# blackpigg/MCMTT_OPTICALFLOW

Hardware: AMD Instinct MI355X
Metric: Tracker2D frames/sec (all cameras) + achieved HBM GB/s fraction, 1/2/4/8 GPU (higher is better)
Workload: dtype u8+f32

## Files before the change

include/psn_lk.h:

```cpp
#ifndef PSN_LK_H
#define PSN_LK_H

#include <stddef.h>
#include <stdint.h>

#ifdef __cplusplus
extern "C" {
#endif

#define PSN_LK_ABI_VERSION 5

#define PSN_LK_OK 0
#define PSN_LK_ERR_ARG (-1)
#define PSN_LK_ERR_WINSIZE (-2)
#define PSN_LK_ERR_HIP (-3)
#define PSN_LK_ERR_NOMEM (-4)
#define PSN_LK_ERR_SLOT (-5)
#define PSN_LK_ERR_LEVEL_CAP (-6)
#define PSN_LK_ERR_COMM (-7)
#define PSN_LK_ERR_UNSUPPORTED (-8)

#define PSN_LK_USE_INITIAL_FLOW 4
#define PSN_LK_GET_MIN_EIGENVALS 8
#define PSN_LK_ACCUM_SCALAR 0x100
// ... 54 lines not shown
int psn_lk_track(psn_lk_ctx *ctx, const psn_lk_query *q, int nq, const float *prev_xy, float *next_xy,
                 uint8_t *status, float *err);
int psn_lk_track_device(psn_lk_ctx *ctx, const psn_lk_query *q, int nq, const float *d_prev_xy,
                        float *d_next_xy, uint8_t *d_status, float *d_err);

int psn_lk_track_device_counted(psn_lk_ctx *ctx, const psn_lk_query *q, int nq, const int *d_counts,
                                const float *d_prev_xy, float *d_next_xy, uint8_t *d_status, float *d_err);
int psn_lk_track_device_counted_strided(psn_lk_ctx *ctx, const psn_lk_query *q, int nq, const int *d_counts,
                                        int count_stride, const float *d_prev_xy, float *d_next_xy, uint8_t *d_status,
                                        float *d_err);

int psn_calc_optical_flow_pyr_lk(psn_lk_ctx *ctx, const uint8_t *prev_img, const uint8_t *next_img,
                                 int stride, const float *prev_pts, float *next_pts, uint8_t *status,
                                 float *err, int npts, const psn_lk_params *params);

int psn_lk_read_level(psn_lk_ctx *ctx, int slot, int level, uint8_t *host, int stride);
int psn_lk_level_size(psn_lk_ctx *ctx, int level, int *w, int *h);

int psn_lk_enable_timing(psn_lk_ctx *ctx, int capacity, int every);
int psn_lk_timing_stats(psn_lk_ctx *ctx, int *n_push, double *push_ms, int *n_track, double *track_ms);
int psn_lk_timing_launches(psn_lk_ctx *ctx, int cap, double *ms, int *tag, int *n);

#define PSN_LK_VARIANT_THREADS 1
#define PSN_LK_VARIANT_GENERIC 2
#define PSN_LK_VARIANT_ONEWAVE 3
#define PSN_LK_VARIANT_BOX 4
#define PSN_LK_VARIANT_TILED_LDS 5
#define PSN_LK_VARIANT_FUSED_HELPERS 6
#define PSN_LK_VARIANT_LARGE 7
#define PSN_LK_VARIANT_LG_LDS 8
#define PSN_LK_VARIANT_LG_JR 9
#define PSN_LK_VARIANT_ST_OVL 10
#define PSN_LK_VARIANT_POISON_LDS 11
int psn_lk_debug_set_variant(psn_lk_ctx *ctx, int key, int value);

int psn_lk_debug_count_samples(psn_lk_ctx *ctx, int on);
int psn_lk_debug_read_samples(psn_lk_ctx *ctx, unsigned long long *out);

int psn_lk_debug_set_stamps(psn_lk_ctx *ctx, void *d_stamps);

typedef struct psn_gridfast_params {
    int threshold;
    int nonmax;
    int max_total;
    int grid_rows;
    int grid_cols;
    int cap;
} psn_gridfast_params;
void psn_gridfast_default_params(psn_gridfast_params *p);
int psn_gridfast_detect(psn_lk_ctx *ctx, int slot, const int *rois, int nroi, const psn_gridfast_params *p,
                        uint32_t seed, float *out_xy, int *out_count, int *out_total);
int psn_gridfast_detect_device(psn_lk_ctx *ctx, int slot, const int *rois, int nroi, const psn_gridfast_params *p,
                               uint32_t seed, float *d_out_xy, int *d_out_count, int *d_out_total);
int psn_gridfast_detect_device_sets(psn_lk_ctx *ctx, int nset, const int *slots, const int *nrois, const int *rois,
                                    const psn_gridfast_params *p, uint32_t seed, float *d_out_xy, int *d_out_count,
                                    int *d_out_total);

#define PSN_RGBHIST_BINS 16
typedef struct psn_rgbhist_rect {
    const uint8_t *frame;
    int stride;
    int x, y, w, h;
} psn_rgbhist_rect;
int psn_rgbhist_device(const psn_rgbhist_rect *d_rects, int nrect, uint32_t *d_counts, void *hip_stream);
int psn_lk_box_histograms(psn_lk_ctx *ctx, int nset, const int *slots, const int *nrects, const int *rects,
                          uint32_t *counts);
// ... 19 lines not shown
```

mcmtt_opticalflow_amd/_lib.py:

```python
from __future__ import annotations

import ctypes
import os
import re

_HERE = os.path.dirname(os.path.abspath(__file__))
LIB_PATH = os.path.join(_HERE, "lib", "libpsn_lk.so")
STAMPS_LIB_PATH = os.path.join(_HERE, "lib", "libpsn_lk_stamps.so")
HEADER_PATH = os.path.join(os.path.dirname(_HERE), "include", "psn_lk.h")
HEADER_PATHS = [HEADER_PATH] + [os.path.join(os.path.dirname(_HERE), "include", h)
                                for h in ("psn_sgsmooth.h", "psn_t2d_device.h", "psn_jpeg.h")]

PSN_LK_OK = 0
ERRORS = {
    -1: "PSN_LK_ERR_ARG",
    -2: "PSN_LK_ERR_WINSIZE",
    -3: "PSN_LK_ERR_HIP",
    -4: "PSN_LK_ERR_NOMEM",
    -5: "PSN_LK_ERR_SLOT",
    -6: "PSN_LK_ERR_LEVEL_CAP",
    -7: "PSN_LK_ERR_COMM",
    -8: "PSN_LK_ERR_UNSUPPORTED",
}
USE_INITIAL_FLOW = 4
GET_MIN_EIGENVALS = 8
ACCUM_SCALAR = 0x100
OVERLAP_OFF, OVERLAP_STREAM, OVERLAP_FUSED = 0, 1, 2
TERM_COUNT = 1
TERM_EPS = 2
MAX_WIN_WIDTH = 6400
COMM_UNIQUE_ID_BYTES = 128
VARIANTS = {"threads": 1, "generic": 2, "onewave": 3, "box": 4, "tiled_lds": 5, "fused_helpers": 6,
            "large": 7, "lg_lds": 8, "lg_jr": 9, "st_ovl": 10, "poison_lds": 11}


class PsnLkError(RuntimeError):
    def __init__(self, code: int, msg: str = ""):
        self.code = code
        super().__init__(f"{ERRORS.get(code, code)}: {msg}")


class LkParams(ctypes.Structure):
    _fields_ = [
        ("win_w", ctypes.c_int),
        ("win_h", ctypes.c_int),
        ("max_level", ctypes.c_int),
        ("term_type", ctypes.c_int),
        ("max_count", ctypes.c_int),
        ("epsilon", ctypes.c_double),
        ("flags", ctypes.c_int),
        ("min_eig_threshold", ctypes.c_double),
    ]


class LkQuery(ctypes.Structure):
    _fields_ = [
        ("prev_slot", ctypes.c_int),
        ("next_slot", ctypes.c_int),
        ("first_pt", ctypes.c_int),
        ("num_pts", ctypes.c_int),
        ("params", LkParams),
    ]


class GridFastParams(ctypes.Structure):
    _fields_ = [
# ... 164 lines not shown
```

mcmtt_opticalflow_amd/csrc/psn_lk_abi.cpp:

```cpp
#include <hip/hip_runtime.h>
#include <hsa/hsa.h>
#include <hsa/hsa_ext_amd.h>

#include <algorithm>
#include <chrono>
#include <mutex>
#include <cstdarg>
#include <cstdio>
#include <cstdlib>
#include <cstring>
#include <new>
#include <string>
#include <vector>

#include "psn_lk.h"
#include "psn_jpeg.h"
#include "psn_gridfast.h"
#include "psn_rgbhist.h"
#include "psn_lk_kernels.h"

using psn::LevelDev;

struct psn_lk_ctx {
    int device = 0;
// ... 33 lines not shown
    struct ColorSrc {
        const uint8_t *p = nullptr;
        int stride = 0, channels = 0;
        bool shared = false;
        unsigned gen = 0;
    };
    std::vector<ColorSrc> color_src;
    unsigned src_gen = 0;
    hipStream_t hist_stream = nullptr;
    hipEvent_t hist_ev = nullptr;
    psn_rgbhist_rect *h_hist_rects = nullptr;
    psn_rgbhist_rect *d_hist_rects = nullptr;
    uint32_t *h_hist_counts = nullptr;
    uint32_t *d_hist_counts = nullptr;
    size_t hist_cap = 0;
    psn_jpeg_ctx *jpeg = nullptr;
    uint8_t *d_pyr = nullptr;
    LevelDev *d_slots = nullptr;
    std::vector<LevelDev> h_slots;
    std::vector<char> filled;
    uint8_t *d_src = nullptr;
    size_t d_src_cap = 0;
    float *d_prev = nullptr, *d_next = nullptr, *d_err = nullptr;
    uint8_t *d_status = nullptr;
    size_t d_pts_cap = 0;
    int force_threads = 0;
    bool force_generic = false;
    bool onewave = true;
#ifndef PSN_ST_OVL_DEFAULT
#define PSN_ST_OVL_DEFAULT 1
#endif
    bool st_ovl = PSN_ST_OVL_DEFAULT != 0;
    bool poison_lds = false;
    bool box = true;
    int tiled_lds = 76 * 1024;
    int num_cus = 256;
    bool force_large = false;
    int lg_lds = 24 * 1024;
    bool lg_jr = true;
    struct LgWs {
        hipStream_t s = nullptr;
        void *p = nullptr;
        size_t bytes = 0;
        hipEvent_t done = nullptr;
    };
    std::vector<LgWs> lg_ws;
    std::vector<void *> lg_retired;
    unsigned long long *d_stamps = nullptr;
    unsigned long long *d_samples = nullptr;
    bool count_samples = false;
    uint32_t *d_gf_kp = nullptr;
    int *d_gf_cnt = nullptr;
    size_t gf_kp_cap = 0, gf_cnt_cap = 0;
    float *d_gf_xy = nullptr;
    int *d_gf_oc = nullptr, *d_gf_ot = nullptr;
    size_t gf_out_cap = 0;
    int gf_nroi_cap = 0;
    int tcap = 0;
    std::vector<hipEvent_t> ev_push, ev_track;
    std::vector<int> track_tag;
    long n_push = 0, n_track = 0;
    long calls_push = 0, calls_track = 0;
    int every = 1;
    std::string err;
};

// ... 870 lines not shown
        bool builds = false;
        if (c->pend && fused_slot < 0 && !d_counts) {
            int tx, ty, plds;
            psn::pyramid_grid(c->pend_args, tx, ty, plds);
            a.pyr = c->pend_args;
            a.pyr_ntiles = tx * ty;
            a.pyr_tiles_x = tx;
            a.pyr_ctr = c->d_ctr;
            const int helpers = std::min(c->fused_helpers, a.pyr_ntiles);
            a.lk_wgs = wgs;
            a.total_wgs = wgs + helpers;
            wgs += helpers;
            lds = std::max(lds, psn::kStScratchBytes + plds);
            c->pend = false;
            fused_slot = c->pend_slot;
            builds = true;
        }
        a.poison_lds = c->poison_lds ? lds : 0;
        HIPCHK(c, psn::launch_lk_st(a, wgs, nt, ept, ow_e, occ, lds, c->stream));
        return builds ? mark_fused_build(c, fused_slot) : PSN_LK_OK;
    }
    if (cls == kClsBx) {
        const int upt = key / 10;
        const bool notail = key % 10 != 0;
        int lds_bx = 0;
        for (int i = 0; i < a.nq; i++) {
            psn::LkQueryDev &d = a.q[i];
            d.bx_hw = 1;
            while (d.bx_hw < 8 && psn::BxLayout(d.win_w, d.win_h, upt, d.bx_hw + 1).total <= psn::bx_lds_target(upt, notail))
                d.bx_hw++;
            lds_bx = std::max(lds_bx, psn::BxLayout(d.win_w, d.win_h, upt, d.bx_hw).total);
        }
        a.poison_lds = c->poison_lds ? lds_bx : 0;
        HIPCHK(c, psn::launch_lk_bx(a, wgs, upt, notail, lds_bx, c->stream));
        return PSN_LK_OK;
    }
    if (cls == kClsTiled) {
        int threads = maxpx <= 1024 ? 64 : maxpx <= 4096 ? 128 : 256;
        if (forced == 64 || forced == 128 || forced == 256) threads = forced;
        lds = 0;
        for (int i = 0; i < a.nq; i++) lds = std::max(lds, psn::lk_lds_bytes(a.q[i].win_w, a.q[i].win_h, a.q[i].tile_rows));
        HIPCHK(c, psn::launch_lk(a, wgs, threads, lds, c->stream));
        return PSN_LK_OK;
    }
    long long slot = 0;
    lds = 0;
    for (int i = 0; i < a.nq; i++) {
        slot = std::max(slot, psn::lg_slot_int2(a.q[i].win_w, a.q[i].win_h));
        lds = std::max(lds, psn::lg_lds_bytes(a.q[i].win_w, a.q[i].win_h, a.q[i].tile_rows, a.q[i].lg_jr != 0, key));
    }
    const size_t slot_bytes = (size_t)slot * 8;
    const long long fit = std::max<long long>((long long)(kLgWsBudget / slot_bytes), 1);
    const int grid = (int)std::min<long long>(wgs, fit);
    void *ws = nullptr;
    int rc = ensure_lg_ws(c, slot_bytes * grid, &ws);
    if (rc) return rc;
    a.lg_ws = (int2 *)ws;
    a.lg_slot = slot;
    a.lk_wgs = wgs;
    a.total_wgs = wgs;
    a.poison_lds = c->poison_lds ? lds : 0;
    HIPCHK(c, psn::launch_lk_lg(a, grid, lds, key, c->stream));
    for (auto &e : c->lg_ws)
        if (e.s == c->stream) {
            if (!e.done) HIPCHK(c, hipEventCreateWithFlags(&e.done, hipEventDisableTiming));
            HIPCHK(c, hipEventRecord(e.done, c->stream));
// ... 228 lines not shown
    if (!prev_pts || !next_pts || !status) return PSN_LK_ERR_ARG;
    HIPCHK(c, hipSetDevice(c->device));
    const int sa = c->user_slots, sb = c->user_slots + 1;
    int rc = push_host_impl(c, sa, prev_img, stride, 1);
    if (rc) return rc;
    rc = push_host_impl(c, sb, next_img, stride, 1);
    if (rc) return rc;
    psn_lk_query q;
    q.prev_slot = sa;
    q.next_slot = sb;
    q.first_pt = 0;
    q.num_pts = npts;
    q.params = p;
    return track_host_impl(c, &q, 1, prev_pts, next_pts, status, err, true);
}

int psn_lk_debug_set_variant(psn_lk_ctx *c, int key, int value) {
    if (!c) return PSN_LK_ERR_ARG;
    switch (key) {
    case PSN_LK_VARIANT_THREADS:
        if (value != 0 && value != 64 && value != 128 && value != 256 && value != 512) return PSN_LK_ERR_ARG;
        c->force_threads = value;
        return PSN_LK_OK;
    case PSN_LK_VARIANT_GENERIC: c->force_generic = value != 0; return PSN_LK_OK;
    case PSN_LK_VARIANT_ONEWAVE: c->onewave = value != 0; return PSN_LK_OK;
    case PSN_LK_VARIANT_BOX: c->box = value != 0; return PSN_LK_OK;
    case PSN_LK_VARIANT_TILED_LDS: c->tiled_lds = std::max(16 * 1024, std::min(value, 160 * 1024 - 1024)); return PSN_LK_OK;
    case PSN_LK_VARIANT_FUSED_HELPERS: c->fused_helpers = std::max(0, value); return PSN_LK_OK;
    case PSN_LK_VARIANT_LARGE: c->force_large = value != 0; return PSN_LK_OK;
    case PSN_LK_VARIANT_LG_LDS: c->lg_lds = std::max(4 * 1024, std::min(value, 160 * 1024 - 1024)); return PSN_LK_OK;
    case PSN_LK_VARIANT_LG_JR: c->lg_jr = value != 0; return PSN_LK_OK;
    case PSN_LK_VARIANT_ST_OVL: c->st_ovl = value != 0; return PSN_LK_OK;
    case PSN_LK_VARIANT_POISON_LDS: c->poison_lds = value != 0; return PSN_LK_OK;
    default: return PSN_LK_ERR_ARG;
    }
}

int psn_lk_debug_count_samples(psn_lk_ctx *c, int on) {
    if (!c) return PSN_LK_ERR_ARG;
    HIPCHK(c, hipSetDevice(c->device));
    if (on) {
        if (!c->d_samples) HIPCHK(c, hipMalloc(&c->d_samples, sizeof(unsigned long long)));
        HIPCHK(c, hipDeviceSynchronize());
        HIPCHK(c, hipMemset(c->d_samples, 0, sizeof(unsigned long long)));
    }
    c->count_samples = on != 0;
    return PSN_LK_OK;
}

int psn_lk_debug_read_samples(psn_lk_ctx *c, unsigned long long *out) {
    if (!c || !out) return PSN_LK_ERR_ARG;
    *out = 0;
    if (!c->d_samples) return PSN_LK_OK;
    HIPCHK(c, hipSetDevice(c->device));
    HIPCHK(c, hipDeviceSynchronize());
    HIPCHK(c, hipMemcpy(out, c->d_samples, sizeof(unsigned long long), hipMemcpyDeviceToHost));
    return PSN_LK_OK;
}

int psn_lk_debug_set_stamps(psn_lk_ctx *c, void *d_stamps) {
    if (!c) return PSN_LK_ERR_ARG;
#ifdef PSN_LK_STAMPS
    c->d_stamps = (unsigned long long *)d_stamps;
    return PSN_LK_OK;
#else
    (void)d_stamps;
// ... 273 lines not shown
```

mcmtt_opticalflow_amd/csrc/psn_lk_kernels.h:

```cpp
#pragma once

#include <hip/hip_runtime.h>
#include <stdint.h>

#include "psn_lk.h"

namespace psn {

constexpr int kMaxLevels = PSN_LK_MAX_LEVELS;
constexpr int kMaxQueries = 32;
constexpr int kJMargin = 3;
constexpr int kPyrMaxTop = 5;

struct LevelDev {
    uint8_t *p;
    int w, h, pitch;
    int pad_;
};

struct PyrBuildArgs {
    const uint8_t *src;
    int src_stride;
    int channels;
    int nlevels;
// ... 26 lines not shown
    int sub_pts, sub_pstride;
};
__device__ __forceinline__ int lk_query_point(const LkQueryDev &Q, const int *counts, int count_stride, int g) {
    int loc = g - Q.wg_begin;
    if (Q.sub_pts > 0) {
        const int sub = loc / Q.sub_pts;
        loc -= sub * Q.sub_pts;
        if (counts && loc >= counts[Q.qidx + sub * count_stride]) return -1;
        return Q.pt_begin + sub * Q.sub_pstride + loc;
    }
    if (counts && loc >= counts[Q.qidx]) return -1;
    return Q.pt_begin + loc;
}
__host__ __device__ inline unsigned div_magic(int d) { return d > 0 ? ((1u << 22) + (unsigned)d - 1u) / (unsigned)d : 0u; }

struct RingGeo {
    uint8_t *base;
    long long slot_bytes;
    long long off[kMaxLevels];
    int w[kMaxLevels], h[kMaxLevels], pitch[kMaxLevels];
};

struct LkLaunchArgs {
    const LevelDev *slots;
    RingGeo ring;
    const float *prev;
    float *next;
    uint8_t *status;
    float *err;
    unsigned long long *stamps;
    unsigned long long *samples;
    int nq;
    int poison_lds;
    const int *counts;
    int count_stride;
    LkQueryDev q[kMaxQueries];
    int pyr_ntiles, pyr_tiles_x;
    int total_wgs, lk_wgs;
    unsigned *pyr_ctr;
    PyrBuildArgs pyr;
    int2 *lg_ws;
    long long lg_slot;
};

__host__ __device__ constexpr int align16(int x) { return (x + 15) & ~15; }
__host__ __device__ inline int lk_jreg_w(int w) { return w + 1 + 2 * kJMargin; }
__host__ __device__ inline int lk_jreg_h(int h) { return h + 1 + 2 * kJMargin; }
__host__ __device__ inline int lk_off_dw(int w, int h) { return align16(2 * w * h); }
__host__ __device__ inline int lk_off_jr(int w, int h) { return lk_off_dw(w, h) + align16(4 * w * h); }
__host__ __device__ inline int lk_off_red(int w, int h) { return lk_off_jr(w, h) + align16(lk_jreg_w(w) * lk_jreg_h(h)); }
constexpr int kRedBytes = 256;
__host__ __device__ inline int lk_off_tile(int w, int h) { return lk_off_red(w, h) + kRedBytes; }
__host__ __device__ inline int lk_tile_pimg_bytes(int w, int tr) { return align16((tr + 3) * (w + 3)); }
__host__ __device__ inline int lk_tile_dg_bytes(int w, int tr) { return align16(4 * (tr + 1) * (w + 1)); }
__host__ __device__ inline int lk_tile_prod_bytes(int w, int tr) { return 12 * (tr * w + 20); }
__host__ __device__ inline int lk_lds_bytes(int w, int h, int tr) {
    return lk_off_tile(w, h) + lk_tile_pimg_bytes(w, tr) + lk_tile_dg_bytes(w, tr) + lk_tile_prod_bytes(w, tr);
}

__host__ __device__ inline int round16i(int x) { return (x + 15) & ~15; }
__host__ __device__ inline int lk_st_planeA(int w, int h, bool sse) {
    const int n = sse ? w / 4 : 0;
    return 4 * round16i(h * n) + round16i(h * (w - 4 * n) + 1);
}
__host__ __device__ inline int lk_st_planeB(int w, int h, bool sse) {
    const int n = sse ? w / 8 : 0;
// ... 56 lines not shown
            iw = dg + nlev * dg_stride;
            r = iw + nlev * iw_stride;
            ra = r;
            int rb = rb_a;
            if (rb < pb) rb = pb;
            if (rb < eb) rb = eb;
            total = r + rb;
        }
    }
};
constexpr int kBxNT = 256;
constexpr int kBxMaxUPT = 16;
constexpr int kBxRecInts = 8 * 15 + 4;
constexpr int kBxXInts = 2 * 4 * kBxRecInts;
constexpr int kBxScrBytes = (kBxXInts + 32) * 4 + 64;
constexpr int kBxMaxLds = 64 * 1024;
constexpr int kBxMaxLds2 = 80 * 1024;
constexpr int kBxLdsTarget = 53 * 1024;
__host__ __device__ constexpr int bx_occupancy(int upt, bool notail) {
    return upt <= 4 ? 4 : (upt >= 12 || (!notail && upt >= 10)) ? 2 : 3;
}
__host__ __device__ constexpr int bx_lds_target(int upt, bool notail) {
    return bx_occupancy(upt, notail) == 4 ? 40 * 1024 : bx_occupancy(upt, notail) == 3 ? kBxLdsTarget : kBxMaxLds2;
}
__host__ __device__ constexpr int bx_max_lds(int upt, bool notail) {
    return bx_occupancy(upt, notail) == 2 ? kBxMaxLds2 : kBxMaxLds;
}
__host__ __device__ inline int bx_qw(int w) { return (w + 3) >> 2; }
__host__ __device__ inline int bx_pm(int w) { return bx_qw(w) + 2; }
__host__ __device__ inline int bx_jrp(int w) { return st_jreg_w(w) + 8; }
__host__ __device__ inline int bx_round4(int x) { return (x + 3) & ~3; }
__host__ __device__ inline int bx_region(int n) { return ((n + 15) & ~15) + 4; }
__host__ __device__ inline int bx_pc(int upt) { return 128 * upt + 96; }
struct BxLayout {
    int jr, un, pb, total;
    __host__ __device__ BxLayout(int w, int h, int upt, int hw = 1) {
        jr = align16(kBxScrBytes);
        un = jr + align16(st_jreg_h(h) * bx_jrp(w));
        const int pim = align16((h + 3) * 4 * bx_pm(w));
        const int planes = 24 * bx_pc(upt) * hw;
        pb = pim > planes ? pim : planes;
        total = un + pb + 1024;
    }
};
inline int bx_err_rows(int w, int h, int pb) {
    for (int t = h; t >= 1; t--)
        if (4 * bx_round4(t * w) <= pb) return t;
    return 1;
}

constexpr int kLgNT = 256;
constexpr int kLgTQs[2] = {192, 128};
constexpr int kLgTQNoJr = 128;
constexpr int kLgTQE = 128;
__host__ __device__ constexpr int lg_sreg(int tq) { return ((tq + 15) & ~15) + 4; }
__host__ __device__ constexpr int lg_plane(int tq) { return 4 * lg_sreg(tq) + ((4 * tq + 15) & ~15) + 4; }
__host__ __device__ constexpr int lg_scr_bytes() { return align16((kBxXInts + 32) * 4); }
__host__ __device__ constexpr int lg_tiles_a_bytes(int tq) { return 2 * 3 * lg_plane(tq) * 4 + 1024; }
__host__ __device__ constexpr int lg_tiles_b_bytes(int tq) { return 2 * 2 * lg_plane(tq) * 4 + 1024; }
__host__ __device__ inline int lg_band_bytes(int w, int tr) { return align16((tr + 3) * 4 * bx_pm(w)); }
__host__ __device__ inline int lg_jr_bytes(int w, int h) { return align16(st_jreg_h(h) * bx_jrp(w)); }
#ifndef PSN_LG_XB
#define PSN_LG_XB 0
#endif
constexpr int kXbRecBytes = 10 * 256 * 8;
#ifndef PSN_LG_POOL_KB
// ... 68 lines not shown
```

mcmtt_opticalflow_amd/csrc/psn_lk_kernels.hip:

```cpp
#include <float.h>
#include <limits.h>

#include <type_traits>

#include "psn_gridfast.h"
#include "psn_lk_kernels.h"
#include "psn_lk_device.h"
#include "psn_lk_bx.h"

namespace psn {


#define LK_STAMP(slot) PSN_STAMP(A.stamps, threadIdx.x == 0, (size_t)blockIdx.x * 64 + (slot))
#define LK_COUNT(slot, v) PSN_STAMP_VAL(A.stamps, threadIdx.x == 0, (size_t)blockIdx.x * 64 + (slot), v)




__device__ __forceinline__ uint8_t load_src(const PyrBuildArgs &a, int y, int x) {
    const uint8_t *row = a.src + (size_t)y * a.src_stride;
    if (a.channels == 1) return row[x];
    const uint8_t *p = row + 3 * x;
    return (uint8_t)((p[0] * 1868 + p[1] * 9617 + p[2] * 4899 + (1 << 13)) >> 14);
}
// ... 1671 lines not shown
        A.status[pi] = (uint8_t)status;
        if (A.err) A.err[pi] = errv;
    }
    if (A.pyr_ntiles > 0) pyr_tail<NT>(A, smem);
}

template <int UPT, bool NOTAIL>
__global__ __launch_bounds__(kBxNT, bx_occupancy(UPT, NOTAIL)) void lk_kernel_bx(LkLaunchArgs A) {
    extern __shared__ __attribute__((aligned(16))) uint8_t smem[];
    static_assert(UPT % 2 == 0, "units are processed in pairs");
    constexpr int NT = kBxNT;
    const int tid = threadIdx.x, lane = tid & 63;
    if (A.poison_lds) lds_poison<NT>(smem, A.poison_lds);
    const int g = xcd_remap((int)blockIdx.x, (int)gridDim.x);
    int qi = 0;
    while (qi + 1 < A.nq && g >= A.q[qi + 1].wg_begin) qi++;
    const LkQueryDev &Q = A.q[qi];
    const int pi = lk_query_point(Q, A.counts, A.count_stride, g);
    if (pi < 0) return;
    const int w = Q.win_w, h = Q.win_h;
    const int maxL = Q.max_level, flags = Q.flags;
    const bool sse = (flags & PSN_LK_ACCUM_SCALAR) == 0;
    const int QW = bx_qw(w), U = h * QW;
    const int nqB = sse ? (w / 8) * 2 : 0, n8 = 4 * nqB, tB = w - n8;
    const int nqA = sse ? w / 4 : 0, nA4 = 4 * nqA, tA = w - nA4;
    const int PM = bx_pm(w), JRW = st_jreg_w(w), JRH = st_jreg_h(h), JRP = bx_jrp(w), JRP4 = JRP >> 2;
    const BxLayout lay(w, h, UPT);
    int *X = (int *)smem;
    float *RS = (float *)(X + kBxXInts);
    int *EP = (int *)(RS + 16);
    volatile int *FLG = (volatile int *)(RS + 24);
    if (threadIdx.x < 7) FLG[threadIdx.x] = threadIdx.x < 6 ? -1 : 0;
    int fb_epoch = 0;
    uint8_t *JR = smem + lay.jr;
    const uint32_t *JR32 = (const uint32_t *)JR;
    uint8_t *UN = smem + lay.un;
    const uint32_t *P32 = (const uint32_t *)UN;
    float *PL = (float *)UN;

    const int u0 = tid * UPT;
    const int y0 = u0 / QW, q0 = u0 - y0 * QW;
    unsigned UB[UPT / 2];
    unsigned sseB = 0;
    {
        int y = y0, q = q0;
#pragma unroll
        for (int k = 0; k < UPT; k++) {
            const unsigned o = u0 + k < U ? (unsigned)(y * JRP + 4 * q) : 0u;
            if (k & 1)
                UB[k >> 1] |= o << 16;
            else
                UB[k >> 1] = o;
            sseB |= (unsigned)(q < nqB) << k;
            if (++q == QW) {
                q = 0;
                y++;
            }
        }
    }

    const float hwx = __fmul_rn((float)(w - 1), 0.5f), hwy = __fmul_rn((float)(h - 1), 0.5f);
    const float px0 = A.prev[2 * pi], py0 = A.prev[2 * pi + 1];
    float NPx = 0.f, NPy = 0.f;
    if (flags & PSN_LK_USE_INITIAL_FLOW) {
        NPx = A.next[2 * pi];
        NPy = A.next[2 * pi + 1];
    }
    int status = 1;
    float errv = 0.f;
    int par = 0;
#ifdef PSN_LK_STAMPS
    unsigned long long bx_acc[16] = {}, bx_t = 0, bx_t0 = 0, bx_r0 = 0;
    PSN_CLK_ORDERED(bx_t0);
    bx_t = bx_t0;
    asm volatile("s_memrealtime %0\n\ts_waitcnt lgkmcnt(0)" : "=s"(bx_r0) : : "memory");
#endif

    unsigned IP[UPT][2], XP[UPT][2], YP[UPT][2];
    int gmax = 0;
    unsigned nwin = 0;

    for (int level = maxL; level >= 0; level--) {
        const LevelDev I = ring_level_u(A.ring, Q.prev_slot, level);
        const LevelDev J = ring_level_u(A.ring, Q.next_slot, level);
        const int cols = I.w, rows = I.h;
        const float scale = ldexpf(1.f, -level);
        float px = __fmul_rn(px0, scale), py = __fmul_rn(py0, scale);
        float nx, ny;
        if (level == maxL) {
            if (flags & PSN_LK_USE_INITIAL_FLOW) {
                nx = __fmul_rn(NPx, scale);
                ny = __fmul_rn(NPy, scale);
            } else {
                nx = px;
                ny = py;
            }
        } else {
            nx = __fmul_rn(NPx, 2.f);
            ny = __fmul_rn(NPy, 2.f);
        }
        NPx = nx;
        NPy = ny;
        px = __fsub_rn(px, hwx);
        py = __fsub_rn(py, hwy);
        const int ipx = cv_floor(px), ipy = cv_floor(py);
        if (win_outside(ipx, ipy, w, h, cols, rows)) {
            if (level == 0) {
                status = 0;
                errv = 0.f;
            }
            continue;
        }
        int iw00, iw01, iw10, iw11;
        bilin_weights(__fsub_rn(px, (float)ipx), __fsub_rn(py, (float)ipy), iw00, iw01, iw10, iw11);
        nx = __fsub_rn(nx, hwx);
        ny = __fsub_rn(ny, hwy);
        int jr_x0 = (cv_floor(nx) - kStJMargin) & ~3, jr_y0 = cv_floor(ny) - kStJMargin;

        __syncthreads();
        dma_patch<NT>(UN, I, ipy - 1, ipx - 1, w + 3, h + 3, PM, Q.dv_bxpm);
        dma_wait();
        dma_patch<NT>(JR, J, jr_y0, jr_x0, JRW, JRH, JRP4, Q.dv_bxjr);
        barrier_inflight();
        PSN_PH_MARK(bx_acc, bx_t, 0);
        bx_prio_lo();

        float sA[3];
        nwin++;
        {
            const int sh = (ipx - 1) & 3;
            int T11[5] = {0, 0, 0, 0, 0}, T22[5] = {0, 0, 0, 0, 0}, T12[5] = {0, 0, 0, 0, 0};
            int M12[5] = {0, 0, 0, 0, 0}, m12[5] = {0, 0, 0, 0, 0};
            int gmx = 0, gmn = 0;
            const bool interior = ipx >= 0 && ipy >= 0 && ipx + 4 * QW + 2 <= cols && ipy + h + 1 <= rows;
            const int c256 = 1 << 8, c8192 = 1 << 13;
            auto apass = [&](auto inner) {
            constexpr bool IN = decltype(inner)::value;
            int y = y0, q = q0;
            asm volatile("" : "+v"(y), "+v"(q));
#pragma unroll
            for (int k = 0; k < UPT; k++) {
                const bool uv = u0 + k < U;
                const int yy = uv ? y : 0, qq = uv ? q : 0;
                bx_unit<IN, NOTAIL>(P32, PM, sh, yy, qq, uv, w, ipx, ipy, cols, rows, iw00, iw01, iw10, iw11, c256,
                                    c8192, IP[k], XP[k], YP[k], gmx, gmn);
                asm volatile("" : "+v"(IP[k][0]), "+v"(IP[k][1]), "+v"(XP[k][0]), "+v"(XP[k][1]), "+v"(YP[k][0]),
                             "+v"(YP[k][1]), "+v"(gmx), "+v"(gmn));
                if (++q == QW) {
                    q = 0;
                    y++;
                }
                __builtin_amdgcn_sched_barrier(0);
            }
            };
            if (interior)
                apass(std::true_type());
            else
                apass(std::false_type());
            gmax = max(gmx, -gmn);
            int q = q0;
// ... 39 lines not shown
                            T22[4] = mad16p<1, 1>(yt[u][hh], yt[u][hh], mad16p<0, 0>(yt[u][hh], yt[u][hh], T22[4]));
                            const int ta = mad16p<0, 0>(xt[u][hh], yt[u][hh], T12[4]);
                            const int tb = mad16p<1, 1>(xt[u][hh], yt[u][hh], ta);
                            run2(T12[4], M12[4], m12[4], ta, tb);
                        }
                }
                asm volatile("" : "+v"(T11[0]), "+v"(T11[1]), "+v"(T11[2]), "+v"(T11[3]), "+v"(T11[4]), "+v"(T22[0]),
                             "+v"(T22[1]), "+v"(T22[2]), "+v"(T22[3]), "+v"(T22[4]));
                asm volatile("" : "+v"(T12[0]), "+v"(T12[1]), "+v"(T12[2]), "+v"(T12[3]), "+v"(T12[4]), "+v"(M12[0]),
                             "+v"(M12[1]), "+v"(M12[2]), "+v"(M12[3]), "+v"(M12[4]));
                asm volatile("" : "+v"(m12[0]), "+v"(m12[1]), "+v"(m12[2]), "+v"(m12[3]), "+v"(m12[4]));
            }
            int T[15], M[15], m[15];
#pragma unroll
            for (int c = 0; c < 5; c++) {
                T[c] = T11[c], M[c] = T11[c], m[c] = 0;
                T[5 + c] = T12[c], M[5 + c] = M12[c], m[5 + c] = m12[c];
                T[10 + c] = T22[c], M[10 + c] = T22[c], m[10 + c] = 0;
            }
            PSN_PH_MARK(bx_acc, bx_t, 1);
            bx_prio_hi();
            int *rec = X + par * 4 * kBxRecInts;
            par ^= 1;
            bx_publish<15>(T, rec, NOTAIL || tA == 0);
            dma_wait();
            __syncthreads();
            bx_check<15>(T, M, m, false, rec, NOTAIL || tA == 0);
            __syncthreads();
            int tot, h0, base0;
            const bool exact = bx_eval<15>(rec, tot, h0, base0);
            if (exact) {
#pragma unroll
                for (int s = 0; s < 3; s++) sA[s] = combine_a5([&](int i) { return rl_f(tot, i); }, s, sse);
            } else {
                int ftid = (int)threadIdx.x;
                asm volatile("" : "+v"(ftid));
                const int HW = Q.bx_hw, PCA = 3 * bx_pc(UPT) * HW;
                const bool chl = ftid < 15;
                const int cl = chl ? ftid : 0, cs = cl / 5, cc = cl - 5 * cs;
                float acc = (float)base0;
                const int g_last = (U - 1) / (32 * UPT);
                auto geoA = [&](int g, int &sa, int &ta, int &nsse, int &ntail) {
                    const int ua = 32 * UPT * g, ub = min(ua + 32 * UPT * HW, U);
                    sa = (ua / QW) * nqA + min(ua % QW, nqA);
                    ta = (ua / QW) * tA + min(max(4 * (ua % QW) - nA4, 0), tA);
                    nsse = (ub / QW) * nqA + min(ub % QW, nqA) - sa;
                    ntail = (ub / QW) * tA + min(max(4 * (ub % QW) - nA4, 0), tA) - ta;
                };
                auto unitA = [&](int yk, int qk, bool uv, unsigned x0, unsigned x1, unsigned y0_, unsigned y1_, float *buf,
                                 int S, int P, int sa, int ta) {
                    if (!uv) return;
                    unsigned xp[2] = {x0, x1}, yp[2] = {y0_, y1_};
                    asm volatile("" : "+v"(xp[0]), "+v"(xp[1]), "+v"(yp[0]), "+v"(yp[1]));
                    const bool su = NOTAIL || qk < nqA;
                    const int base = su ? yk * nqA + qk - sa : 4 * S + yk * tA + 4 * qk - nA4 - ta;
#pragma unroll
                    for (int i = 0; i < 4; i++) {
                        const int gx = (i & 1) ? hi16(xp[i >> 1]) : lo16(xp[i >> 1]);
                        const int gy = (i & 1) ? hi16(yp[i >> 1]) : lo16(yp[i >> 1]);
                        const bool on = 4 * qk + i < w;
                        float *d1 = on ? buf + (su ? i * S + base : base + i) : PL + 2 * PCA;
                        const int pp = on ? P : 1;
                        d1[0] = (float)__mul24(gx, gx);
                        d1[pp] = (float)__mul24(gx, gy);
                        d1[2 * pp] = (float)__mul24(gy, gy);
                    }
// ... 108 lines not shown
                    for (int i = len; i < ((len + 15) & ~15); i++) rg[i] = 0.f;
                };
                writeA(h0, PL);
                padA(h0, PL);
                __syncthreads();
                for (int g = h0, t = 0; g <= g_last; g += HW, t ^= 1) {
                    float *cur = PL + t * PCA, *nxt = PL + (t ^ 1) * PCA;
                    if (g + HW <= g_last) writeA(g + HW, nxt);
                    if ((ftid >> 6) == 0) {
                        int sa, ta, nsse, ntail;
                        geoA(g, sa, ta, nsse, ntail);
                        const int S = bx_region(nsse), P = 4 * S + bx_region(ntail);
                        const int len = chl ? (cc < 4 ? nsse : ntail) : 0;
                        const int nbmax = NOTAIL ? (nsse + 15) >> 4 : __builtin_amdgcn_readlane(wave_max_scan((len + 15) >> 4), 63);
                        if (chl && (!NOTAIL || cc < 4)) acc = chain_sum_pl<NOTAIL>(cur + cs * P + cc * S, len, nbmax, acc);
                        if (g + HW <= g_last) padA(g + HW, nxt);
                    }
                    __syncthreads();
                }
                if (ftid < 64) {
#pragma unroll
                    for (int s = 0; s < 3; s++) {
                        const float t = combine_a5([&](int i) { return readlane_f(acc, i); }, s, sse);
                        if (ftid == 0) RS[s] = t;
                    }
                }
                __syncthreads();
                sA[0] = RS[0];
                sA[1] = RS[1];
                sA[2] = RS[2];
            }
            PSN_PH_MARK(bx_acc, bx_t, 2);
        }
        const LkSolve S = lk_solve(sA[0], sA[1], sA[2], w * h, Q.min_eig);
        if (flags & PSN_LK_GET_MIN_EIGENVALS) errv = S.minEig;
        if (!S.ok) {
            if (level == 0) status = 0;
            continue;
        }

        float pdx = 0.f, pdy = 0.f;
        for (int j = 0; j < Q.max_count; j++) {
            const int inx = cv_floor(nx), iny = cv_floor(ny);
            if (win_outside(inx, iny, w, h, cols, rows)) {
                if (level == 0) status = 0;
                break;
            }
            int w00, w01, w10, w11;
            bilin_weights(__fsub_rn(nx, (float)inx), __fsub_rn(ny, (float)iny), w00, w01, w10, w11);
            if (!(jr_covers(inx, iny, w, h, jr_x0, jr_y0, JRW, JRH))) {
                jr_x0 = (inx - kStJMargin) & ~3;
                jr_y0 = iny - kStJMargin;
                dma_patch<NT>(JR, J, jr_y0, jr_x0, JRW, JRH, JRP4, Q.dv_bxjr);
                dma_wait();
                __syncthreads();
            }
            PSN_PH_MARK(bx_acc, bx_t, 3);
            bx_prio_lo();
            PSN_PH_COUNT(bx_acc, 10);
            nwin++;
            const unsigned W0 = pack_w(w00, w01), W1 = pack_w(w10, w11);
            const int ox = inx - jr_x0, oy = iny - jr_y0, sj = ox & 3;
            const unsigned s0 = bx_sel(sj, 0), s1 = bx_sel(sj, 1), s2 = bx_sel(sj, 2), s3 = bx_sel(sj, 3);
            int T1[5] = {0, 0, 0, 0, 0}, M1[5] = {0, 0, 0, 0, 0}, m1[5] = {0, 0, 0, 0, 0};
            int T2[5] = {0, 0, 0, 0, 0}, M2[5] = {0, 0, 0, 0, 0}, m2[5] = {0, 0, 0, 0, 0};
            int dmx = 0, dmn = 0;
            const int c256 = opaque256();
            const bool dtrack = __ballot(gmax > kExact / 8160) != 0ull;
            auto bmain = [&](auto trk) {
                unsigned jo0 = (unsigned)((const uint8_t *)(JR32 + oy * JRP4 + (ox >> 2)) - smem);
                unsigned jo1 = jo0 + 4u * (unsigned)JRP4;
// ... 84 lines not shown
                    asm volatile("" : "+v"(T1[0]), "+v"(T1[1]), "+v"(T1[2]), "+v"(T1[3]), "+v"(T1[4]), "+v"(M1[0]),
                                 "+v"(M1[1]), "+v"(M1[2]), "+v"(M1[3]), "+v"(M1[4]));
                    asm volatile("" : "+v"(m1[0]), "+v"(m1[1]), "+v"(m1[2]), "+v"(m1[3]), "+v"(m1[4]), "+v"(T2[0]),
                                 "+v"(T2[1]), "+v"(T2[2]), "+v"(T2[3]), "+v"(T2[4]));
                    asm volatile("" : "+v"(M2[0]), "+v"(M2[1]), "+v"(M2[2]), "+v"(M2[3]), "+v"(M2[4]), "+v"(m2[0]),
                                 "+v"(m2[1]), "+v"(m2[2]), "+v"(m2[3]), "+v"(m2[4]), "+v"(dmx), "+v"(dmn));
                }
            };
            if (dtrack)
                bmain(std::true_type());
            else
                bmain(std::false_type());
            const int dmax = max(dmx, -dmn);
            const bool bad = (long long)dmax * gmax > (long long)kExact;
            int T[10], M[10], m[10];
#pragma unroll
            for (int c = 0; c < 5; c++) {
                T[c] = T1[c], M[c] = M1[c], m[c] = m1[c];
                T[5 + c] = T2[c], M[5 + c] = M2[c], m[5 + c] = m2[c];
            }
            PSN_PH_MARK(bx_acc, bx_t, 4);
            bx_prio_hi();
            int *rec = X + par * 4 * kBxRecInts;
            par ^= 1;
            bx_publish<10>(T, rec, NOTAIL || tB == 0);
            PSN_PH_MARK(bx_acc, bx_t, 9);
            __syncthreads();
            bx_check<10>(T, M, m, bad, rec, NOTAIL || tB == 0);
            __syncthreads();
            int tot, h0, base0;
            float b1, b2;
            const bool bex = bx_eval<10>(rec, tot, h0, base0);
            PSN_PH_MARK(bx_acc, bx_t, 5);
            if (bex) {
                combine_b10([&](int i) { return rl_f(tot, i); }, sse, b1, b2);
            } else {
                int ftid = (int)threadIdx.x;
                asm volatile("" : "+v"(ftid));
                const int HW = Q.bx_hw, PC = bx_pc(UPT) * HW;
                const bool chl = ftid < 10;
                const int cl = chl ? ftid : 0, cs = cl / 5, cc = cl - 5 * cs;
                float acc = (float)base0;
                const int g_last = (U - 1) / (32 * UPT);
                auto tile_geo = [&](int g, int &sa, int &ta, int &nsse, int &ntail) {
                    const int ua = 32 * UPT * g, ub = min(ua + 32 * UPT * HW, U);
                    sa = (ua / QW) * nqB + min(ua % QW, nqB);
                    ta = (ua / QW) * tB + min(max(4 * (ua % QW) - n8, 0), tB);
                    nsse = (ub / QW) * nqB + min(ub % QW, nqB) - sa;
                    ntail = (ub / QW) * tB + min(max(4 * (ub % QW) - n8, 0), tB) - ta;
                };
                auto tile_unit = [&](int yk, int qk, bool uv, const unsigned (&ip)[2], const unsigned (&xp)[2],
                                     const unsigned (&yp)[2], float *buf, int S, int P, int sa, int ta, int zf) {
                    if (!uv) return;
                    int d[4];
                    bx_diffs(JR32 + (oy + yk) * JRP4 + (ox >> 2) + qk, JRP4, W0, W1, s0, s1, s2, s3, ip, d, zf);
                    const bool su = NOTAIL || qk < nqB;
                    const int base = su ? yk * nqB + qk - sa : 4 * S + yk * tB + 4 * qk - n8 - ta;
#pragma unroll
                    for (int i = 0; i < 4; i++) {
                        const int gx = (i & 1) ? hi16(xp[i >> 1]) : lo16(xp[i >> 1]);
                        const int gy = (i & 1) ? hi16(yp[i >> 1]) : lo16(yp[i >> 1]);
                        const bool on = 4 * qk + i < w;
                        float *d1 = on ? buf + (su ? i * S + base : base + i) : PL + 6 * PC;
                        d1[0] = (float)__mul24(d[i], gx);
                        d1[on ? P : 1] = (float)__mul24(d[i], gy);
                    }
                };
                constexpr int K1 = UPT / 2;
                const bool split = HW == 1 && (UPT & 1) == 0;
// ... 278 lines not shown
                                if (4 * qk + i < w) PL[(yk - r0) * w + 4 * qk + i] = (float)abs(d[i]);
                        }
                        if (++qk == QW) {
                            qk = 0;
                            yk++;
                        }
                    }
                    __syncthreads();
                    if (tid == 0) acc = chain_sum(PL, tr * w, acc);
                }
                if (tid == 0) RS[8] = acc;
                __syncthreads();
                errval = RS[8];
            }
            errv = lk_err(errval, w * h);
        }
    }

#ifdef PSN_LK_STAMPS
    {
        unsigned long long t_end;
        PSN_CLK_ORDERED(t_end);
        bx_acc[15] = t_end - bx_t0;
        unsigned long long r1;
        unsigned hwid, xcc;
        asm volatile("s_memrealtime %0\n\ts_waitcnt lgkmcnt(0)" : "=s"(r1) : : "memory");
        asm volatile("s_getreg_b32 %0, hwreg(HW_REG_HW_ID)" : "=s"(hwid));
        asm volatile("s_getreg_b32 %0, hwreg(HW_REG_XCC_ID)" : "=s"(xcc));
        if (tid == 0 && A.stamps) {
            for (int i = 0; i < 16; i++) A.stamps[(size_t)g * 64 + i] = bx_acc[i];
            A.stamps[(size_t)g * 64 + 16] = bx_r0;
            A.stamps[(size_t)g * 64 + 17] = r1;
            A.stamps[(size_t)g * 64 + 18] = ((unsigned long long)xcc << 32) | hwid;
        }
    }
#endif
    if (tid == 0) {
        if (FLG[6]) {
            NPx = NPy = errv = __builtin_nanf("");
            status = 0;
        }
        A.next[2 * pi] = NPx;
        A.next[2 * pi + 1] = NPy;
        A.status[pi] = (uint8_t)status;
        if (A.err) A.err[pi] = errv;
        if (A.samples) atomicAdd(A.samples, (unsigned long long)nwin * (unsigned)(w * h));
    }
}

#define PSN_BX_KERNELS(X)                                         \
    X(4, true) X(4, false) X(8, true) X(8, false) X(10, true)     \
    X(10, false) X(12, true) X(12, false) X(16, true) X(16, false)
#define PSN_ST_KERNELS(X)                                                                 \
    X(64, 2, 0, 1) X(64, 4, 0, 1) X(128, 2, 0, 1) X(128, 4, 0, 1) X(256, 2, 0, 1)         \
    X(512, 1, 0, 1) X(512, 2, 0, 1) X(256, 2, 4, 1) X(256, 2, 7, 1) X(256, 2, 8, 1)       \
    X(256, 4, 8, 1) X(256, 2, 16, 1) X(256, 4, 16, 1) X(256, 4, 0, 1) X(256, 2, 4, 3)     \
    X(256, 2, 7, 3) X(256, 2, 8, 3)

hipError_t launch_lk_bx(const LkLaunchArgs &a, int total_wgs, int upt, bool notail, int lds_bytes, hipStream_t s) {
    if (total_wgs <= 0) return hipSuccess;
    const dim3 grid(total_wgs), block(kBxNT);
#define PSN_BX_LAUNCH(U, NOTAIL)                                                         \
    if (upt == U && notail == NOTAIL) {                                                  \
        hipLaunchKernelGGL((lk_kernel_bx<U, NOTAIL>), grid, block, lds_bytes, s, a);     \
        return hipGetLastError();                                                        \
    }
// ... 47 lines not shown
```

Baseline: 2600.

## Defer inexact A-matrix fallback and fuse it with first-iteration b-vector pass

When the fast exact path for the structure tensor (A) fails in the box LK kernel, the fallback tile reduction is now deferred and merged into the first iteration's b-vector fallback. One double-buffered LDS tile pass computes all five gradient products (gx², gxgy, gy², d·gx, d·gy) together. The goal is to avoid two separate slow tile sweeps over the window gradients on the fallback path. The change is controlled by a new default-on bx_fuse variant and a compile-time LDS-fit check. It adds code complexity, LDS usage and a different loop exit (break) when the solve fails.

After: 2612, median of 6. About the same (+0.5%).

```diff
diff --git a/include/psn_lk.h b/include/psn_lk.h
--- a/include/psn_lk.h
+++ b/include/psn_lk.h
@@ -110,6 +110,7 @@
 #define PSN_LK_VARIANT_LG_JR 9
 #define PSN_LK_VARIANT_ST_OVL 10
 #define PSN_LK_VARIANT_POISON_LDS 11
+#define PSN_LK_VARIANT_BX_FUSE 12
 int psn_lk_debug_set_variant(psn_lk_ctx *ctx, int key, int value);
 
 int psn_lk_debug_count_samples(psn_lk_ctx *ctx, int on);
diff --git a/mcmtt_opticalflow_amd/_lib.py b/mcmtt_opticalflow_amd/_lib.py
--- a/mcmtt_opticalflow_amd/_lib.py
+++ b/mcmtt_opticalflow_amd/_lib.py
@@ -31,7 +31,7 @@
 MAX_WIN_WIDTH = 6400
 COMM_UNIQUE_ID_BYTES = 128
 VARIANTS = {"threads": 1, "generic": 2, "onewave": 3, "box": 4, "tiled_lds": 5, "fused_helpers": 6,
-            "large": 7, "lg_lds": 8, "lg_jr": 9, "st_ovl": 10, "poison_lds": 11}
+            "large": 7, "lg_lds": 8, "lg_jr": 9, "st_ovl": 10, "poison_lds": 11, "bx_fuse": 12}
 
 
 class PsnLkError(RuntimeError):
diff --git a/mcmtt_opticalflow_amd/csrc/psn_lk_abi.cpp b/mcmtt_opticalflow_amd/csrc/psn_lk_abi.cpp
--- a/mcmtt_opticalflow_amd/csrc/psn_lk_abi.cpp
+++ b/mcmtt_opticalflow_amd/csrc/psn_lk_abi.cpp
@@ -89,6 +89,10 @@
 #endif
     bool st_ovl = PSN_ST_OVL_DEFAULT != 0;
     bool poison_lds = false;
+#ifndef PSN_BX_FUSE_DEFAULT
+#define PSN_BX_FUSE_DEFAULT 1
+#endif
+    bool bx_fuse = PSN_BX_FUSE_DEFAULT != 0;
     bool box = true;
     int tiled_lds = 76 * 1024;
     int num_cus = 256;
@@ -1025,6 +1029,7 @@
             lds_bx = std::max(lds_bx, psn::BxLayout(d.win_w, d.win_h, upt, d.bx_hw).total);
         }
         a.poison_lds = c->poison_lds ? lds_bx : 0;
+        a.bx_fuse = c->bx_fuse ? 1 : 0;
         HIPCHK(c, psn::launch_lk_bx(a, wgs, upt, notail, lds_bx, c->stream));
         return PSN_LK_OK;
     }
@@ -1319,6 +1324,7 @@
     case PSN_LK_VARIANT_LG_JR: c->lg_jr = value != 0; return PSN_LK_OK;
     case PSN_LK_VARIANT_ST_OVL: c->st_ovl = value != 0; return PSN_LK_OK;
     case PSN_LK_VARIANT_POISON_LDS: c->poison_lds = value != 0; return PSN_LK_OK;
+    case PSN_LK_VARIANT_BX_FUSE: c->bx_fuse = value != 0; return PSN_LK_OK;
     default: return PSN_LK_ERR_ARG;
     }
 }
diff --git a/mcmtt_opticalflow_amd/csrc/psn_lk_kernels.h b/mcmtt_opticalflow_amd/csrc/psn_lk_kernels.h
--- a/mcmtt_opticalflow_amd/csrc/psn_lk_kernels.h
+++ b/mcmtt_opticalflow_amd/csrc/psn_lk_kernels.h
@@ -82,6 +82,7 @@
     unsigned long long *samples;
     int nq;
     int poison_lds;
+    int bx_fuse;
     const int *counts;
     int count_stride;
     LkQueryDev q[kMaxQueries];
@@ -204,6 +205,11 @@
 __host__ __device__ inline int bx_round4(int x) { return (x + 3) & ~3; }
 __host__ __device__ inline int bx_region(int n) { return ((n + 15) & ~15) + 4; }
 __host__ __device__ inline int bx_pc(int upt) { return 128 * upt + 96; }
+__host__ __device__ inline int bx_fz_plane(int n) { return 4 * bx_region(n) + 4; }
+__host__ __device__ inline int bx_fz_buf(int n) { return 5 * bx_fz_plane(n); }
+__host__ __device__ constexpr bool bx_fz_build(int upt, bool notail) {
+    return notail && 48 * (128 * upt + 96) + kBxScrBytes <= bx_lds_target(upt, notail);
+}
 struct BxLayout {
     int jr, un, pb, total;
     __host__ __device__ BxLayout(int w, int h, int upt, int hw = 1) {
diff --git a/mcmtt_opticalflow_amd/csrc/psn_lk_kernels.hip b/mcmtt_opticalflow_amd/csrc/psn_lk_kernels.hip
--- a/mcmtt_opticalflow_amd/csrc/psn_lk_kernels.hip
+++ b/mcmtt_opticalflow_amd/csrc/psn_lk_kernels.hip
@@ -1727,6 +1727,11 @@
     volatile int *FLG = (volatile int *)(RS + 24);
     if (threadIdx.x < 7) FLG[threadIdx.x] = threadIdx.x < 6 ? -1 : 0;
     int fb_epoch = 0;
+    constexpr bool FZ = bx_fz_build(UPT, NOTAIL);
+    int *DA = (int *)(RS + 32);
+    auto fz_fits = [&]() {
+        return A.bx_fuse && Q.max_count > 0 && 8 * bx_fz_buf(32 * UPT) <= BxLayout(w, h, UPT, Q.bx_hw).pb;
+    };
     uint8_t *JR = smem + lay.jr;
     const uint32_t *JR32 = (const uint32_t *)JR;
     uint8_t *UN = smem + lay.un;
@@ -1765,7 +1770,7 @@
     float errv = 0.f;
     int par = 0;
 #ifdef PSN_LK_STAMPS
-    unsigned long long bx_acc[16] = {}, bx_t = 0, bx_t0 = 0, bx_r0 = 0;
+    unsigned long long bx_acc[24] = {}, bx_t = 0, bx_t0 = 0, bx_r0 = 0;
     PSN_CLK_ORDERED(bx_t0);
     bx_t = bx_t0;
     asm volatile("s_memrealtime %0\n\ts_waitcnt lgkmcnt(0)" : "=s"(bx_r0) : : "memory");
@@ -1821,6 +1826,7 @@
         bx_prio_lo();
 
         float sA[3];
+        bool defA = false;
         nwin++;
         {
             const int sh = (ipx - 1) & 3;
@@ -1926,6 +1932,11 @@
             if (exact) {
 #pragma unroll
                 for (int s = 0; s < 3; s++) sA[s] = combine_a5([&](int i) { return rl_f(tot, i); }, s, sse);
+            } else if (FZ && fz_fits() && !win_outside(cv_floor(nx), cv_floor(ny), w, h, cols, rows)) {
+                defA = true;
+                int dt = (int)threadIdx.x;
+                asm volatile("" : "+v"(dt));
+                if (dt < 16) DA[dt] = dt < 15 ? base0 : h0;
             } else {
                 int ftid = (int)threadIdx.x;
                 asm volatile("" : "+v"(ftid));
@@ -2100,11 +2111,14 @@
             }
             PSN_PH_MARK(bx_acc, bx_t, 2);
         }
-        const LkSolve S = lk_solve(sA[0], sA[1], sA[2], w * h, Q.min_eig);
-        if (flags & PSN_LK_GET_MIN_EIGENVALS) errv = S.minEig;
-        if (!S.ok) {
-            if (level == 0) status = 0;
-            continue;
+        LkSolve S = {};
+        if (!defA) {
+            S = lk_solve(sA[0], sA[1], sA[2], w * h, Q.min_eig);
+            if (flags & PSN_LK_GET_MIN_EIGENVALS) errv = S.minEig;
+            if (!S.ok) {
+                if (level == 0) status = 0;
+                continue;
+            }
         }
 
         float pdx = 0.f, pdy = 0.f;
@@ -2255,9 +2269,128 @@
             float b1, b2;
             const bool bex = bx_eval<10>(rec, tot, h0, base0);
             PSN_PH_MARK(bx_acc, bx_t, 5);
-            if (bex) {
-                combine_b10([&](int i) { return rl_f(tot, i); }, sse, b1, b2);
-            } else {
+            if (bex) combine_b10([&](int i) { return rl_f(tot, i); }, sse, b1, b2);
+            bool fzd = false;
+            if constexpr (FZ) if (defA) {
+                defA = false;
+                fzd = true;
+                int ftid = (int)threadIdx.x;
+                asm volatile("" : "+v"(ftid));
+                constexpr int K1 = UPT / 2;
+                constexpr int TU = 32 * UPT;
+                const int BUF = bx_fz_buf(TU);
+                const int t0a = DA[15], t0b = bex ? 1 << 20 : h0;
+                const int t_first = min(t0a, t0b), t_last = (U - 1) / TU;
+                const bool chl = ftid < 20;
+                const int cl = chl ? ftid : 0, cp = cl >> 2, ci = cl & 3;
+                const int bA = DA[5 * min(cp, 2) + ci];
+                const int bB = __builtin_amdgcn_ds_bpermute(4 * (5 * max(cp - 3, 0) + ci), base0);
+                const float acc0 = (float)(cp < 3 ? bA : bB);
+                const int tst = cp < 3 ? t0a : t0b;
+                float acc = acc0;
+                unsigned fo0 = (unsigned)((const uint8_t *)(JR32 + oy * JRP4 + (ox >> 2)) - smem);
+                unsigned fo1 = fo0 + 4u * (unsigned)JRP4;
+                asm volatile("" : "+s"(fo0), "+s"(fo1));
+                auto fz_write = [&](int g, float *buf, auto lowerT) {
+                    constexpr bool lower = decltype(lowerT)::value;
+                    const int zf = opaque256();
+                    const int n = min(TU, U - g * TU), S = bx_region(n), P = bx_fz_plane(n);
+                    const bool up = (ftid & 32) != 0;
+                    const int ub = lower ? (up ? (ftid ^ 32) * UPT + K1 : ftid * UPT) : (up ? ftid * UPT + K1 : (ftid ^ 32) * UPT);
+                    const int rel = ub - g * TU;
+                    const bool wb = g >= t0b;
+                    auto pick = [](unsigned a, unsigned b) {
+                        auto r = __builtin_amdgcn_permlane32_swap(a, b, false, false);
+                        return lower ? r[0] : r[1];
+                    };
+                    auto uoff = [&](int k) { return (k & 1) ? UB[k >> 1] >> 16 : UB[k >> 1] & 0xffffu; };
+#pragma unroll
+                    for (int k = 0; k < K1; k++) {
+                        const unsigned ip[2] = {pick(IP[k][0], IP[K1 + k][0]), pick(IP[k][1], IP[K1 + k][1])};
+                        unsigned xp[2] = {pick(XP[k][0], XP[K1 + k][0]), pick(XP[k][1], XP[K1 + k][1])};
+                        unsigned yp[2] = {pick(YP[k][0], YP[K1 + k][0]), pick(YP[k][1], YP[K1 + k][1])};
+                        const unsigned off = pick(uoff(k), uoff(K1 + k));
+                        if (ub + k < U) {
+                            asm volatile("" : "+v"(xp[0]), "+v"(xp[1]), "+v"(yp[0]), "+v"(yp[1]));
+                            float *d1 = buf + rel + k;
+#pragma unroll
+                            for (int i = 0; i < 4; i++) {
+                                const int gx = (i & 1) ? hi16(xp[i >> 1]) : lo16(xp[i >> 1]);
+                                const int gy = (i & 1) ? hi16(yp[i >> 1]) : lo16(yp[i >> 1]);
+                                d1[i * S] = (float)__mul24(gx, gx);
+                                d1[i * S + P] = (float)__mul24(gx, gy);
+                                d1[i * S + 2 * P] = (float)__mul24(gy, gy);
+                            }
+                            if (wb) {
+                                int d[4];
+                                bx_diffs2((const uint32_t *)(smem + fo0 + off), (const uint32_t *)(smem + fo1 + off), W0, W1,
+                                          s0, s1, s2, s3, ip, d, zf);
+#pragma unroll
+                                for (int i = 0; i < 4; i++) {
+                                    const int gx = (i & 1) ? hi16(xp[i >> 1]) : lo16(xp[i >> 1]);
+                                    const int gy = (i & 1) ? hi16(yp[i >> 1]) : lo16(yp[i >> 1]);
+                                    d1[i * S + 3 * P] = (float)__mul24(d[i], gx);
+                                    d1[i * S + 4 * P] = (float)__mul24(d[i], gy);
+                                }
+                            }
+                        }
+                    }
+                };
+                for (int g = t_first - 1, t = 1; g <= t_last; g++, t ^= 1) {
+                    float *cur = PL + t * BUF, *nxt = PL + (t ^ 1) * BUF;
+                    if (g < t_last && (ftid >> 6) == (g + 1) >> 1) {
+                        if ((g + 1) & 1)
+                            fz_write(g + 1, nxt, std::false_type());
+                        else
+                            fz_write(g + 1, nxt, std::true_type());
+                    }
+                    if (chl) {
+                        if (g >= t_first) {
+                            const int n = min(TU, U - g * TU);
+                            acc = chain_sum_pl<true>(cur + cp * bx_fz_plane(n) + ci * bx_region(n), n, (n + 15) >> 4, acc);
+                            if (g < tst) acc = acc0;
+                        }
+                        if (g < t_last) {
+                            const int n = min(TU, U - (g + 1) * TU);
+                            float *rg = nxt + cp * bx_fz_plane(n) + ci * bx_region(n);
+                            for (int i = n; i < ((n + 15) & ~15); i++) rg[i] = 0.f;
+                        }
+                    }
+                    __syncthreads();
+                }
+                PSN_PH_MARK(bx_acc, bx_t, 19);
+                PSN_PH_COUNT(bx_acc, bex ? 21 : 20);
+                if (ftid < 64) {
+                    auto ga = [&](int i) { return i % 5 == 4 ? 0.f : readlane_f(acc, 4 * (i / 5) + i % 5); };
+#pragma unroll
+                    for (int s = 0; s < 3; s++) {
+                        const float t = combine_a5(ga, s, sse);
+                        if (ftid == 0) RS[s] = t;
+                    }
+                    if (!bex) {
+                        float r1, r2;
+                        combine_b10([&](int i) { return i % 5 == 4 ? 0.f : readlane_f(acc, 12 + 4 * (i / 5) + i % 5); }, sse, r1,
+                                    r2);
+                        if (ftid == 0) {
+                            RS[4] = r1;
+                            RS[5] = r2;
+                        }
+                    }
+                }
+                __syncthreads();
+                if (!bex) {
+                    b1 = RS[4];
+                    b2 = RS[5];
+                }
+                S = lk_solve(RS[0], RS[1], RS[2], w * h, Q.min_eig);
+                if (flags & PSN_LK_GET_MIN_EIGENVALS) errv = S.minEig;
+                if (!S.ok) {
+                    if (level == 0) status = 0;
+                    nwin--;
+                    break;
+                }
+            }
+            if (!fzd && !bex) {
                 int ftid = (int)threadIdx.x;
                 asm volatile("" : "+v"(ftid));
                 const int HW = Q.bx_hw, PC = bx_pc(UPT) * HW;
@@ -2602,6 +2735,7 @@
             A.stamps[(size_t)g * 64 + 16] = bx_r0;
             A.stamps[(size_t)g * 64 + 17] = r1;
             A.stamps[(size_t)g * 64 + 18] = ((unsigned long long)xcc << 32) | hwid;
+            for (int i = 19; i < 22; i++) A.stamps[(size_t)g * 64 + i] = bx_acc[i];
         }
     }
 #endif
```
